# BaptisteHudyma/RGB-D-SLAM

Hardware: AMD Instinct MI355X
Metric: depth frames/s primitive extraction (640x480) (higher is better)
Workload: dtype f64; 1 GPU; 640x480 synthetic planar-room depth stream, plane extraction only (BASELINE.json configs[1]); stream_frames=4096, unique_frames_per_gpu=4096, scene=room, sub_batches=0, frames_rendered_on=device (torch)

## Files before the change

### profiles/a1_inventory.py

```python
#!/usr/bin/env python3
import argparse
import os
import subprocess
import sys

sys.path.insert(0, os.path.dirname(os.path.abspath(__file__)))
from valu_issue import CSRC, RATE_NS, classify, kernel_regions

SYMBOLS = (("f32", "_ZN4cape24cape_cell_moments_kernelILb0EEEvNS_12StageAParamsEi"),
           ("u16", "_ZN4cape24cape_cell_moments_kernelILb1EEEvNS_12StageAParamsEi"))
NAMES = {"prologue": "prologue", "loop_rows_0_9": "rows 0..9, one trip", "row_10": "row 10", "loop_rows_11_18": "rows 11..18, one trip",
         "tail": "tail", "redo_listed": "scan f64 redo"}
ORDER = tuple(NAMES)
WEIGHT = {"prologue": 1, "loop_rows_0_9": 10, "row_10": 1, "loop_rows_11_18": 8, "tail": 1, "redo_listed": 0}


def count(ops):
    c = {"f64": 0, "double_rate": 0, "other": 0}
    for op in ops:
        if op.startswith("v_"):
            c[classify(op)] += 1
    return c


def inventory(asm):
    return {variant: {name: count(ops) for name, ops in kernel_regions(asm, symbol)} for variant, symbol in SYMBOLS}


def priced(c):
# ... 31 lines not shown
```

### profiles/valu_issue.py

```python
#!/usr/bin/env python3
import argparse
import csv
import json
import os
import re
import subprocess
import sys

ROOT = os.path.dirname(os.path.dirname(os.path.abspath(__file__)))
CSRC = os.path.join(ROOT, "rgb-d-slam_amd", "csrc")

RATE_NS = {"f64": 1.95, "other": 1.85, "double_rate": 0.95}
DOUBLE_RATE = {"v_mul_f32", "v_add_f32", "v_sub_f32", "v_subrev_f32", "v_add_u32", "v_sub_u32", "v_subrev_u32", "v_and_b32", "v_mov_b32"}


def classify(op):
    base = re.sub(r"_(e32|e64|dpp|sdwa)$", "", op)
    if "f64" in base or base.endswith("_b64") and base.startswith("v_mov"):
        return "f64"
    if base in DOUBLE_RATE:
        return "double_rate"
    return "other"


def kernel_regions(asm_lines, symbol):
    start = next(i for i, ln in enumerate(asm_lines) if ln.startswith(symbol + ":"))
    end = next(i for i in range(start, len(asm_lines)) if "s_endpgm" in asm_lines[i])
    body = asm_lines[start + 1:end + 1]
    label_at = {m.group(1): i for i, ln in enumerate(body) for m in [re.match(r"^(\.LBB\d+_\d+):", ln)] if m}
    loops = []
    for i, ln in enumerate(body):
        m = re.match(r"\s+s_c?branch\w*\s+(\.LBB\d+_\d+)", ln)
        if m and label_at.get(m.group(1), len(body)) < i:
            loops.append((label_at[m.group(1)], i))
    assert len(loops) == 2, "two row loops"
    redo = []

    def ops(lo, hi):
        out, skip_to = [], None
        for ln in body[lo:hi]:
            if skip_to is not None:
                if ln.startswith(skip_to + ":"):
                    skip_to = None
                else:
                    m = re.match(r"\s+([vs]_\w+)", ln)
                    if m:
                        redo.append(m.group(1))
                    continue
            m = re.match(r"\s+([vs]_\w+|ds_\w+|global_\w+|buffer_\w+|flat_\w+|scratch_\w+)", ln)
            if m:
                out.append(m.group(1))
                v = re.match(r"\s+s_cbranch_vccz\s+(\.LBB\d+_\d+)", ln)
                if v:
                    skip_to = v.group(1)
        return out

    (h1, e1), (h2, e2) = loops
    regions = [("prologue", ops(0, h1)), ("loop_rows_0_9", ops(h1, e1 + 1)), ("row_10", ops(e1 + 1, h2)), ("loop_rows_11_18", ops(h2, e2 + 1)),
               ("tail", ops(e2 + 1, len(body)))]
    return regions + [("redo_listed", redo)]


def count(ops):
    c = {"f64": 0, "double_rate": 0, "other": 0, "salu": 0, "lds": 0, "vmem": 0}
    for op in ops:
        if op.startswith("v_"):
            c[classify(op)] += 1
        elif op.startswith("s_"):
            c["salu"] += 1
        elif op.startswith("ds_"):
            c["lds"] += 1
        else:
            c["vmem"] += 1
    return c
# ... 8 lines not shown
    ap.add_argument("--simds", type=int, default=1024)
    ap.add_argument("--out", default=os.path.join(ROOT, "profiles", "valu_issue.json"))
    args = ap.parse_args()

    asm_path = "/tmp/cape_cell_moments.gfx950.s"
    flags = "-O3 -std=c++17 -fPIC --offload-arch=gfx950 -ffp-contract=off -fno-fast-math -fno-slp-vectorize".split()
    subprocess.check_call(["/opt/rocm/bin/hipcc"] + flags + ["-S", "--cuda-device-only", "-o", asm_path, os.path.join(CSRC, "cape_cell_moments.hip")],
                          stderr=subprocess.DEVNULL)
    asm = open(asm_path).read().splitlines()
    cell = 20
    cells = (args.height // cell) * (args.width // cell)
    waves_per_launch = args.frames * ((cells + 63) // 64)
    out = {"kernel": "cape_cell_moments_kernel", "frames_per_launch": args.frames, "width": args.width, "height": args.height,
           "waves_per_launch": waves_per_launch, "simds": args.simds, "rate_ns_per_wave_instruction": RATE_NS,
           "rates_from": "profiles/r02_valu_rates.txt (csrc/microbench/valu_rates.hip on MI355X)", "variants": {}}
    for variant, symbol in (("f32", "_ZN4cape24cape_cell_moments_kernelILb0EEEvNS_12StageAParamsEi"),
                            ("u16", "_ZN4cape24cape_cell_moments_kernelILb1EEEvNS_12StageAParamsEi")):
        regs = dict(kernel_regions(asm, symbol))
        c = {k: count(v) for k, v in regs.items()}
        weights = {"prologue": 1, "loop_rows_0_9": cell // 2, "row_10": 1, "loop_rows_11_18": cell // 2 - 2, "tail": 1}
        per_wave = {k: sum(c[r][k] * w for r, w in weights.items()) for k in ("f64", "double_rate", "other", "salu", "lds", "vmem")}
        static_valu = per_wave["f64"] + per_wave["double_rate"] + per_wave["other"]
        v = {"static_per_wave": {"all_rows": per_wave, "per_region": {r: c[r] for r in weights}, "redo_listed_not_run": c["redo_listed"],
                                 "per_20_pixels_row_trip": c["loop_rows_0_9"]}}
        valu = static_valu
        if args.pmc:
            for row in csv.DictReader(open(args.pmc)):
                if ("cell_moments_kernel<false>" if variant == "f32" else "cell_moments_kernel<true>") in row["kernel"] and row["counter"] == "SQ_INSTS_VALU":
                    dyn = float(row["avg_value"])
                    v["pmc"] = {"SQ_INSTS_VALU_per_launch": dyn, "per_wave": dyn / waves_per_launch, "static_per_wave": static_valu,
                                "source": os.path.relpath(args.pmc, ROOT)}
                    valu = dyn / waves_per_launch
        mix = {k: per_wave[k] / max(1, static_valu) for k in RATE_NS}
        per_wave_ns = valu * sum(mix[k] * RATE_NS[k] for k in RATE_NS)
        floor_ms = per_wave_ns * waves_per_launch / args.simds * 1e-6
        f64_ns = valu * mix["f64"] * RATE_NS["f64"]
        v.update({"valu_per_wave": valu, "issue_ns_per_wave": per_wave_ns, "floor_ms": floor_ms,
                  "f64_rate_share_of_floor": f64_ns / per_wave_ns,
                  "f64_rate_insts_per_launch": valu * mix["f64"] * waves_per_launch,
                  "other_insts_per_launch": valu * (1.0 - mix["f64"]) * waves_per_launch})
        out["variants"][variant] = v
        print(f"{variant}: per wave (64 cells) f64-rate {per_wave['f64']}, double-rate {per_wave['double_rate']}, other {per_wave['other']} "
              f"= {static_valu} listed, {valu:.0f} priced ({valu / 5:.0f} per 80 pixels per lane); issue floor {floor_ms:.3f} ms per {args.frames} frames "
# ... 8 lines not shown
```

### rgb-d-slam_amd/csrc/cape_api.hip

```cpp
#include <algorithm>
#include <cmath>
#include <cstdlib>
#include <cstring>
#include <initializer_list>
#include <memory>
#include <new>
#include <random>
#include <string>
#include <vector>

#include "cape_handle.h"

using namespace cape::abi;

namespace {

thread_local std::string g_lastError;

constexpr int kRngTableMin = 40000;
int rng_table_size(int cells) { const int need = 43 * cells + 129; return need > kRngTableMin ? need : kRngTableMin; }

std::vector<double> rng_table(uint32_t seed, int count)
{
    std::vector<double> rng((size_t)count);
// ... 15 lines not shown
    const double det = (c00 * m[0][0] + c10 * m[1][0]) + c20 * m[2][0];
    const double invdet = 1.0 / det;
    k00 = c00 * invdet;
    k02 = c20 * invdet;
    k11 = cof(1, 1) * invdet;
    k12 = cof(2, 1) * invdet;
}

struct Knobs
{
    std::string resume;
    bool noResume = false;
    int schedule = 0;
    std::string stageA;
    std::string a1;
    bool growGeneral = false;
    bool pinnedByDma = false;
    int a2WideBatch = 0;
    int generalSlots = 0;
};

int read_knobs(Knobs& k)
{
    auto one_of = [](const char* name, std::initializer_list<const char*> values, std::string& out) {
        const char* e = std::getenv(name);
        if (!e)
            return true;
        out = e;
        return std::any_of(values.begin(), values.end(), [&](const char* v) { return out == v; });
    };
    std::string schedule, grow;
    if (!one_of("CAPE_RESUME", {"off", "wave", "group"}, k.resume))
        return fail(CAPE_ERR_INVALID_ARGUMENT, "CAPE_RESUME must be off, wave or group");
    if (!one_of("CAPE_SCHEDULE", {"two", "single"}, schedule))
        return fail(CAPE_ERR_INVALID_ARGUMENT, "CAPE_SCHEDULE must be two or single");
    if (!one_of("CAPE_STAGE_A", {"strips", "bands"}, k.stageA))
        return fail(CAPE_ERR_INVALID_ARGUMENT, "CAPE_STAGE_A must be strips or bands");
    if (!one_of("CAPE_A1", {"cells", "bands"}, k.a1))
        return fail(CAPE_ERR_INVALID_ARGUMENT, "CAPE_A1 must be cells or bands");
    if (!one_of("CAPE_GROW", {"general", "fast"}, grow))
        return fail(CAPE_ERR_INVALID_ARGUMENT, "CAPE_GROW must be general or fast");
    k.noResume = k.resume == "off" || std::getenv("CAPE_NO_RESUME");
    k.schedule = schedule == "two" ? 1 : (schedule == "single" ? 2 : 0);
    k.growGeneral = grow == "general";
    const char* e = std::getenv("CAPE_PINNED_INPUT");
    k.pinnedByDma = e && std::string(e) == "dma";
    if ((e = std::getenv("CAPE_A2_WIDE_BATCH")))
        k.a2WideBatch = std::atoi(e);
    if ((e = std::getenv("CAPE_GENERAL_SLOTS")))
        k.generalSlots = std::max(1, std::atoi(e));
    return CAPE_OK;
}

template <typename NextFn> int log_frame(cape_log_fn fn, void* user, const cape_frame_record& r, int frame, NextFn next)
// ... 294 lines not shown
    a.brow = h->brow;
    a.ratio_col = h->ratioCol;
    a.ratio_row = h->ratioRow;
    a.cell_sums = h->cellSums;
    a.cell_plane = h->cellPlane;
    a.cell_score = h->cellScore;
    a.cell_tol = h->cellTol;
    a.cell_flags = h->cellFlags;
    a.cell_bins = h->cellBins;
    a.cell_aux = h->cellAux;
    a.cell_mse = h->cellMse;
    a.sinMerge = sinf(static_cast<float>(18.0f * M_PI / 180.0));
    a.cosMergeA = std::cos(static_cast<double>(18.0f) * M_PI / 180.0);
    a.smallBatchFrames = knobs.a2WideBatch;
    a.a1Bands = knobs.a1 == "bands" ? 1 : 0;
    a.minZeroPointCount = static_cast<int>(std::floor(static_cast<float>(400) * 0.7f));

    cape::StageBParams& b = h->pb;
    b.W = cfg->width;
    b.H = cfg->height;
    b.hCells = h->hCells;
    b.vCells = h->vCells;
    b.cells = h->cells;
    b.acol = h->acol;
    b.brow = h->brow;
    b.cell_sums = h->cellSums;
    b.cell_plane = h->cellPlane;
    b.cell_score = h->cellScore;
    b.cell_tol = h->cellTol;
    b.cell_flags = h->cellFlags;
// ... 240 lines not shown
```

### rgb-d-slam_amd/csrc/cape_api_extract.hip

```cpp
#include <algorithm>
#include <atomic>
#include <chrono>
#include <cmath>
#include <cstring>

#include "cape_handle.h"

using namespace cape::abi;

namespace {

__global__ void cape_signal_kernel(uint32_t* flag, uint32_t seq)
{
    __hip_atomic_store(flag, seq, __ATOMIC_RELEASE, __HIP_MEMORY_SCOPE_SYSTEM);
}

void offset_params(const cape_handle_s* h, int f0, cape::StageAParams& a, cape::StageBParams& b)
{
    a = h->pa;
    b = h->pb;
    const size_t C = (size_t)h->cells, F = (size_t)f0;
    const size_t px = F * (size_t)h->cfg.width * h->cfg.height;
    if (a.depth)
        a.depth += px;
// ... 89 lines not shown
    if (t)
        CAPE_HIP_TRY(hipEventRecord(t->e[0], st));
    const bool strips = c.stripCounters && frames <= kHostResultFrames && (!c.inputOverLink || c.stripsAlways);
    cape::StageAParams a2 = a;
    cape::StageBParams bb = b;
    prepare_launch(h, a2, bb, c.spillCounters, strips, frames, t != nullptr);
    if (strips)
    {
        CAPE_HIP_TRY(cape::launch_cell_strips(a2, frames, c.stripCounters, st));
        if (t)
        {
            CAPE_HIP_TRY(hipEventRecord(t->e[1], st));
            CAPE_HIP_TRY(hipEventRecord(t->e[2], st));
        }
    }
    else
    {
        CAPE_HIP_TRY(cape::launch_cell_moments(a, frames, st));
        if (t)
            CAPE_HIP_TRY(hipEventRecord(t->e[1], st));
        CAPE_HIP_TRY(cape::launch_cell_plane(a2, frames, st));
        if (t)
            CAPE_HIP_TRY(hipEventRecord(t->e[2], st));
    }
    const bool oneFrameChain = h->resultsOnHost && r.doneFlag && r.doneCounter && frames <= kHostResultFrames;
    if (oneFrameChain)
    {
        bb.allFrames = c.generalAll ? 0 : 1;
        bb.doneFlag = r.doneFlag;
        bb.doneCounter = r.doneCounter;
// ... 403 lines not shown
```

### rgb-d-slam_amd/csrc/cape_cell_acc.h

```cpp
#pragma once
#include <hip/hip_runtime.h>

#include "cape_device.h"
#include "cape_internal.h"

namespace cape {


#ifndef CAPE_A_GROUP
#define CAPE_A_GROUP 2
#endif
#ifndef CAPE_A_WAVES
#define CAPE_A_WAVES 4
#endif

#ifndef CAPE_A1_CELL_WAVES
#define CAPE_A1_CELL_WAVES 4
#endif
#ifndef CAPE_A1_CELL_THREADS
#define CAPE_A1_CELL_THREADS 256
#endif
#ifndef CAPE_A1_CELL_LOAD_POLICY
#define CAPE_A1_CELL_LOAD_POLICY 0
#endif
constexpr int kThreadsCells = CAPE_A1_CELL_THREADS;
static_assert(kThreadsCells % 64 == 0 && kThreadsCells >= 64 && kThreadsCells <= 1024, "whole waves");

constexpr int kThreadsA = 320;
constexpr int kBandThreads = 160;
[[maybe_unused]] constexpr int kPartStride = 11;

struct PxAcc
// ... 94 lines not shown
```

### rgb-d-slam_amd/csrc/cape_cell_fit.hip

```cpp
#include <hip/hip_runtime.h>

#include <type_traits>

#include "cape_cell_acc.h"

namespace cape {

#ifndef CAPE_A2_WAVES
#define CAPE_A2_WAVES 4
#endif
#ifndef CAPE_A2_ABLATE
#define CAPE_A2_ABLATE 0
#endif
struct CellFit
{
    PlaneFit f;
    bool planar;
    float tol;
    int bin;
    uint32_t nearEdge, inorder, n;
    bool rewrite;
};
__device__ __forceinline__ void cell_fit_and_bin(const StageAParams& p, int frame, int cellRow, int cellCol, const CellAux& aux, double (&S)[9],
                                                 CellFit& o)
{
    PlaneFit f;
    f.planar = false;
    f.nx = f.ny = f.nz = f.d = 0.0;
    f.cx = f.cy = f.cz = 0.0;
    f.mse = kDblMax;
    f.score = 0.0;
    bool planar = false;
    float tol = 0.0f;
    int bin = -1;
    uint32_t nearEdge = 0, inorder = 0;
    uint32_t n = aux.flags & kCountMask;
    const bool continuous = (aux.flags & kAuxContinuous) != 0;
    const bool exact_ok = (aux.flags & kAuxExact) != 0;
    bool rewrite = false;
    if (!exact_ok && continuous && n >= (uint32_t)(kPts / 2))
    {
        inorder = 1;
        rewrite = true;
        const size_t cellOff = (size_t)frame * p.W * p.H + (size_t)(cellRow * kCell) * p.W + cellCol * kCell;
        PxAcc A;
#pragma unroll
        for (int k = 0; k < 9; ++k)
            A.S[k] = 0.0;
        A.n = 0;
        A.zminBits1 = 0;
        A.zmaxBits = 0;
        for (int r = 0; r < kCell; ++r)
        {
            const double b = p.brow[cellRow * kCell + r];
            for (int c = 0; c < kCell; ++c)
            {
                const size_t o = cellOff + (size_t)r * p.W + c;
                const float zr = p.depth ? p.depth[o] : (float)p.depth_u16[o] * p.u16_scale;
                acc_px(zr, p.acol[cellCol * kCell + c], b, A);
            }
        }
#pragma unroll
        for (int k = 0; k < 9; ++k)
            S[k] = A.S[k];
        n = A.n;
    }

    if (!continuous || n < (uint32_t)(kPts / 2))
    {
#pragma unroll
        for (int k = 0; k < 9; ++k)
            S[k] = 0.0;
        n = 0;
        rewrite = true;
    }
    else if (n >= (uint32_t)p.minZeroPointCount && !(CAPE_A2_ABLATE & 1))
    {
        fit_plane(S, n, f);
        const double qz = depth_quantization(f.cz);
        planar = f.mse <= qz * qz;
    }

    if ((CAPE_A2_ABLATE & 1) && n >= (uint32_t)p.minZeroPointCount)
    {
        planar = S[2] > 0.0;
        f.nx = S[0] * 1e-9, f.ny = S[1] * 1e-9, f.nz = -0.5, f.d = S[2] * 1e-6, f.cx = S[0] / n, f.cy = S[1] / n, f.cz = S[2] / n;
    }
    if (planar)
    {
        const float z0 = aux.z0, z1 = aux.z399;
        const int u0 = cellCol * kCell, v0 = cellRow * kCell;
        float x0 = 0, y0 = 0, zz0 = 0, x1 = 0, y1 = 0, zz1 = 0;
        if (z0 > 0)
        {
            x0 = (float)((double)z0 * p.acol[u0]);
            y0 = (float)((double)z0 * p.brow[v0]);
            zz0 = z0;
        }
        if (z1 > 0)
        {
            x1 = (float)((double)z1 * p.acol[u0 + kCell - 1]);
            y1 = (float)((double)z1 * p.brow[v0 + kCell - 1]);
            zz1 = z1;
        }
        const float dx = x1 - x0, dy = y1 - y0, dz = zz1 - zz0;
        const float diam = (CAPE_A2_ABLATE & 8) ? dx : sqrtf(dx * dx + (dy * dy + dz * dz));
        tol = (CAPE_A2_ABLATE & 8) ? diam : std_minf(50.0f, diam * p.sinMerge * sqrtf((float)n));

        const double theta = (CAPE_A2_ABLATE & 2) ? -f.nz : acos(-f.nz);
        const double phi = (CAPE_A2_ABLATE & 2) ? f.nx : atan2(f.nx, f.ny);
        constexpr double kPi = 3.14159265358979323846;
        const double tx = 19.0 * (theta - 0.0) / kPi;
        const int xQ = (int)floor(tx);
        int yQ = 0;
        double ty = 0.5;
        if (xQ > 0)
        {
            ty = 19.0 * (phi - (-kPi)) / (kPi - (-kPi));
            yQ = (int)floor(ty);
        }
        bin = yQ * 20 + xQ;
        if (fabs(tx - rint(tx)) < 1e-9 || (xQ > 0 && fabs(ty - rint(ty)) < 1e-9))
            nearEdge = 1;
    }
    o.f = f;
    o.planar = planar;
    o.tol = tol;
    o.bin = bin;
    o.nearEdge = nearEdge;
    o.inorder = inorder;
    o.n = n;
    o.rewrite = rewrite;
}

struct CellPub
{
    double nx, ny, nz, d, cx, cy, cz, tol;
};

template <int THREADS>
__global__ __launch_bounds__(THREADS, THREADS == 256 ? CAPE_A2_WAVES : 4) void cape_cell_plane_kernel(StageAParams p, int nFrames)
{
    __shared__ CellPub s_pub[THREADS];
    if (blockIdx.x == 0 && threadIdx.x == 0)
    {
        if (p.clear0)
            *p.clear0 = 0u;
        if (p.clear1)
            *p.clear1 = 0u;
        if (p.clear2)
        {
            *p.clear2 = 0u;
            if (p.clear2Buckets)
                for (int c = 1; c <= kResumeClasses; ++c)
                    p.clear2[(size_t)c * p.clear2Buckets] = 0u;
        }
        if (p.clear3)
            *p.clear3 = 0u;
        if (p.clear4)
            p.clear4[0] = p.clear4[1] = 0u;
    }
    const int HC = p.hCells, VC = p.vCells;
    const int rowsPerTile = THREADS / HC > 0 ? THREADS / HC : 1;
    const int tilesPerFrame = (VC + rowsPerTile - 1) / rowsPerTile;
    const int frame = blockIdx.x / tilesPerFrame;
    const int r0 = (blockIdx.x - frame * tilesPerFrame) * rowsPerTile;
    const int tid = threadIdx.x;
    const int tileCells = rowsPerTile * HC;
    const int lrow = tid / HC, cellCol = tid - lrow * HC;
    {
        const int cellRow = r0 + lrow;
        const bool valid = tid < tileCells && cellRow < VC;
        const int cell = cellRow * HC + cellCol;
        const size_t gcell = (size_t)frame * p.cells + (valid ? cell : 0);

        CellFit cf;
// ... 12 lines not shown
            const CellAux aux = p.cell_aux[gcell];
            double* os = p.cell_sums + gcell * kSumStride;
            double S[9];
#pragma unroll
            for (int k = 0; k < 9; ++k)
                S[k] = os[k];
            cell_fit_and_bin(p, frame, cellRow, cellCol, aux, S, cf);
            if (cf.rewrite)
            {
#pragma unroll
                for (int k = 0; k < 9; ++k)
                    os[k] = S[k];
                os[9] = (double)cf.n;
            }
        }
        const PlaneFit& f = cf.f;
        const bool planar = cf.planar;
        const float tol = cf.tol;
        const int bin = cf.bin;
        const uint32_t nearEdge = cf.nearEdge, inorder = cf.inorder, n = cf.n;

        CellPub me;
        me.nx = f.nx; me.ny = f.ny; me.nz = f.nz; me.d = f.d;
        me.cx = f.cx; me.cy = f.cy; me.cz = f.cz; me.tol = (double)tol;
        s_pub[tid] = me;
        __syncthreads();
        uint32_t edges = 0;
        if (valid)
        {
            if (cellCol > 0 && !(CAPE_A2_ABLATE & 4))
            {
                const CellPub L = s_pub[tid - 1];
                if (can_be_merged(L.nx, L.ny, L.nz, L.d, me.nx, me.ny, me.nz, me.cx, me.cy, me.cz, me.tol, p.cosMergeA))
                    edges |= kFlagLeftToMe;
                if (can_be_merged(me.nx, me.ny, me.nz, me.d, L.nx, L.ny, L.nz, L.cx, L.cy, L.cz, L.tol, p.cosMergeA))
                    edges |= kFlagMeToLeft;
            }
            if (lrow > 0 && !(CAPE_A2_ABLATE & 4))
            {
                const CellPub Up = s_pub[tid - HC];
                if (can_be_merged(Up.nx, Up.ny, Up.nz, Up.d, me.nx, me.ny, me.nz, me.cx, me.cy, me.cz, me.tol, p.cosMergeA))
                    edges |= kFlagUpToMe;
                if (can_be_merged(me.nx, me.ny, me.nz, me.d, Up.nx, Up.ny, Up.nz, Up.cx, Up.cy, Up.cz, Up.tol, p.cosMergeA))
                    edges |= kFlagMeToUp;
            }
            double* op = p.cell_plane + gcell * kPlaneStride;
            op[0] = f.nx; op[1] = f.ny; op[2] = f.nz; op[3] = f.d;
            op[4] = f.cx; op[5] = f.cy; op[6] = f.cz; op[7] = f.mse;
            p.cell_mse[gcell] = f.mse;
            p.cell_score[gcell] = f.score;
            p.cell_tol[gcell] = tol;
            p.cell_bins[gcell] = bin;
            p.cell_flags[gcell] = (n & kCountMask) | edges | (nearEdge ? kFlagNearEdge : 0u) | (inorder ? kFlagInorder : 0u) |
                                  (planar ? kFlagPlanar : 0u);
        }
    }
}

constexpr int kStripCells = 8;
constexpr int kStripThreads = 256;
constexpr int kStripCols = kStripCells * 5;
constexpr int kStripRowGroups = 5;
constexpr int kStripRows = kCell / kStripRowGroups;
constexpr int kStripActive = kStripCols * kStripRowGroups;
static_assert(kStripRows * kStripRowGroups == kCell && kStripActive <= kStripThreads, "strip geometry");

__device__ __forceinline__ float4 strip_to_f4(const float4& v, float) { return v; }
__device__ __forceinline__ float4 strip_to_f4(const ushort4& rw, float scale)
{
    auto mul1 = [](float a, float b) {
// ... 5 lines not shown
}

template <bool U16> __global__ __launch_bounds__(kStripThreads) void cape_cell_strip_kernel(StageAParams p, uint32_t* frameCounters)
{
    __shared__ double s_part[kStripActive * kPartStride];
    __shared__ float s_row[kStripCells * kCell];
    __shared__ float s_col[kStripCells * kCell];
    __shared__ float s_corner[kStripCells * 3];
    __shared__ double s_sum[kStripCells * 10];
    __shared__ uint32_t s_range[kStripCells * 2];
    __shared__ uint32_t s_cont[2 * kStripCells];
    __shared__ uint32_t s_last;

    const int t = threadIdx.x;
    if (blockIdx.x == 0 && t == 0)
    {
        if (p.clear0)
            *p.clear0 = 0u;
        if (p.clear1)
            *p.clear1 = 0u;
        if (p.clear2)
        {
            *p.clear2 = 0u;
            if (p.clear2Buckets)
                for (int c = 1; c <= kResumeClasses; ++c)
                    p.clear2[(size_t)c * p.clear2Buckets] = 0u;
        }
        if (p.clear3)
            *p.clear3 = 0u;
        if (p.clear4)
            p.clear4[0] = p.clear4[1] = 0u;
    }
    const int HC = p.hCells, VC = p.vCells;
    const int stripsPerRow = (HC + kStripCells - 1) / kStripCells;
    const int stripsPerFrame = stripsPerRow * VC;
    const int frame = blockIdx.x / stripsPerFrame;
    const int sidx = blockIdx.x - frame * stripsPerFrame;
    const int cellRow = sidx / stripsPerRow;
    const int strip = sidx - cellRow * stripsPerRow;
    const size_t frameOff = (size_t)frame * p.W * p.H;

    const int rg = t / kStripCols;
    const int q = t - rg * kStripCols;
    const int col0 = strip * (kStripCells * kCell) + q * 4;
    const bool active = t < kStripActive && col0 < p.W;
    const int cseg = q / 5, j = q - cseg * 5;

// ... 252 lines not shown
```

### rgb-d-slam_amd/csrc/cape_cell_moments.hip

```cpp
#include <hip/hip_runtime.h>

#include <type_traits>

#include "cape_cell_acc.h"

namespace cape {

template <bool U16> __global__ __launch_bounds__(kThreadsA, CAPE_A_WAVES) void cape_cell_moments_bands_kernel(StageAParams p)
{
    __shared__ double s_part[kThreadsA * kPartStride];
    __shared__ float s_row[64 * kCell];
    __shared__ float s_col[64 * kCell];
    __shared__ float s_corner[64 * 2];
    __shared__ float s_trash[kThreadsA + kCell];

    const int t = threadIdx.x;
    const int frame = blockIdx.x / p.pairsPerFrame;
    const int pair = blockIdx.x - frame * p.pairsPerFrame;
    const size_t frameOff = (size_t)frame * p.W * p.H;

    const int band0 = pair * 2;
    const int cellRow0 = band0 / p.segsPerRow;
    const int seg0 = band0 - cellRow0 * p.segsPerRow;
    const bool wrap = seg0 + 1 == p.segsPerRow;
// ... 221 lines not shown
        }
    }
    const float zmin = __uint_as_float(zminBits1 + 1u), zmax = __uint_as_float(zmaxBits);
    const float rab = fmaxf(p.ratio_col[fCol], p.ratio_row[fRow]);
    const bool exact_ok = zmaxBits <= 0x7F7FFFFFu && ((n == 0) || (zmax * rab <= 512.0f * zmin));

    const size_t gcell = (size_t)frame * p.cells + fRow * p.hCells + fCol;
    CellAux aux;
    aux.z0 = s_corner[c64 * 2];
    aux.z399 = s_corner[c64 * 2 + 1];
    aux.flags = (n & kCountMask) | (continuous ? kAuxContinuous : 0u) | (exact_ok ? kAuxExact : 0u);
    aux.zc = s_row[c64 * kCell + kCell / 2];
    p.cell_aux[gcell] = aux;
}

template <bool U16> __global__ __launch_bounds__(kThreadsCells, CAPE_A1_CELL_WAVES) void cape_cell_moments_kernel(StageAParams p, int nWaves)
{
    const int gw = __builtin_amdgcn_readfirstlane((int)(blockIdx.x * (kThreadsCells / 64) + (threadIdx.x >> 6)));
    if (gw >= nWaves)
        return;
    const int wavesPerFrame = (p.cells + 63) >> 6;
    const int frame = gw / wavesPerFrame;
    const int w = gw - frame * wavesPerFrame;
    const int cell = w * 64 + (int)(threadIdx.x & 63);
    if (cell >= p.cells)
        return;
    const int cellRow = cell / p.hCells;
    const int cellCol = cell - cellRow * p.hCells;
    const size_t frameOff = (size_t)frame * p.W * p.H;

    PxAcc A;
#pragma unroll
    for (int k = 0; k < 9; ++k)
        A.S[k] = 0.0;
    A.n = 0;
    A.zminBits1 = 0xFFFFFFFFu;
    A.zmaxBits = 0u;

    double a[kCell];
    {
        const double2* ap = reinterpret_cast<const double2*>(p.acol + cellCol * kCell);
// ... 135 lines not shown
#pragma unroll
    for (int j = 0; j < kQuads; ++j)
    {
        const float4 v = to_f4(buf[j]);
        acc_piece(v, j, b);
        z399 = v.w;
    }

    const uint32_t n = A.n;
    const float zmin = __uint_as_float(A.zminBits1 + 1u), zmax = __uint_as_float(A.zmaxBits);
    const size_t gcell = my_cell();
    const int ecell = (int)(gcell - (size_t)frame * p.cells);
    int hCells = p.hCells;
    asm volatile("" : "+s"(hCells));
    const int eRow = ecell / hCells;
    const float rab = fmaxf(p.ratio_col[ecell - eRow * hCells], p.ratio_row[eRow]);
    const bool exact_ok = A.zmaxBits <= 0x7F7FFFFFu && ((n == 0) || (zmax * rab <= 512.0f * zmin));

    CellAux aux;
    aux.z0 = z0;
    aux.z399 = z399;
    aux.flags = (n & kCountMask) | (continuous ? kAuxContinuous : 0u) | (exact_ok ? kAuxExact : 0u);
    aux.zc = zc;
    p.cell_aux[gcell] = aux;
    double2* dst = reinterpret_cast<double2*>(p.cell_sums + gcell * kSumStride);
    static_assert(kSumStride == 10, "nine sums and the count: five 16-B stores");
    dst[0] = make_double2(A.S[0], A.S[1]);
    dst[1] = make_double2(A.S[2], A.S[3]);
    dst[2] = make_double2(A.S[4], A.S[5]);
    dst[3] = make_double2(A.S[6], A.S[7]);
    dst[4] = make_double2(A.S[8], (double)n);
}

hipError_t launch_cell_moments(const StageAParams& p, int nFrames, hipStream_t stream)
{
    if (p.a1Bands)
    {
        const int grid = nFrames * p.pairsPerFrame;
        if (p.depth)
            hipLaunchKernelGGL(cape_cell_moments_bands_kernel<false>, dim3(grid), dim3(kThreadsA), 0, stream, p);
        else
            hipLaunchKernelGGL(cape_cell_moments_bands_kernel<true>, dim3(grid), dim3(kThreadsA), 0, stream, p);
        return hipGetLastError();
    }
    constexpr int kWaves = kThreadsCells / 64;
    const int waves = nFrames * ((p.cells + 63) / 64);
    const int grid = (waves + kWaves - 1) / kWaves;
    if (p.depth)
        hipLaunchKernelGGL(cape_cell_moments_kernel<false>, dim3(grid), dim3(kThreadsCells), 0, stream, p, waves);
    else
        hipLaunchKernelGGL(cape_cell_moments_kernel<true>, dim3(grid), dim3(kThreadsCells), 0, stream, p, waves);
    return hipGetLastError();
}

}
```

### rgb-d-slam_amd/csrc/cape_handle.h

```cpp
#pragma once

#include <hip/hip_runtime.h>

#include <cstring>
#include <string>
#include <utility>
#include <vector>

#include "cape_internal.h"

namespace cape {
hipError_t launch_cell_moments(const StageAParams& p, int nFrames, hipStream_t stream);
hipError_t launch_cell_plane(const StageAParams& p, int nFrames, hipStream_t stream);
hipError_t launch_cell_strips(const StageAParams& p, int nFrames, uint32_t* frameCounters, hipStream_t stream);
int cell_plane_rows_per_tile(const StageAParams& p, int nFrames);
hipError_t launch_grow(const StageBParams& p, int nFrames, hipStream_t stream, hipStream_t side, hipEvent_t fork, hipEvent_t done,
                       const GenParams* gen);
hipError_t launch_grow_general(const StageBParams& p, const GenParams& g, int nFrames, hipStream_t stream);
size_t grow_lds_bytes(int cells, bool cylinders, int maxPlanes);
size_t grow_state_bytes(int cells);
bool resume_group_fits(const StageBParams& p);
hipError_t launch_rectify(const RectifyParams& p, int nFrames, int computeUnits, hipStream_t stream);
hipError_t launch_match(const MatchParams& p, int nFrames, hipStream_t stream);
hipError_t launch_pack(const PackParams& p, hipStream_t stream);
hipError_t launch_polygons(const PolygonParams& p, int nFrames, hipStream_t stream);
hipError_t launch_match_polygons(const MatchPolygonParams& p, int nFrames, hipStream_t stream);
hipError_t launch_match_map(const MatchMapParams& p, int nFrames, hipStream_t stream);
hipError_t launch_match_map_wide(const MatchMapParams& p, int nFrames, hipStream_t stream);
hipError_t launch_match_wide(const MatchWideParams& p, int nFrames, hipStream_t stream);
hipError_t launch_carry_save(const CarrySaveParams& p, hipStream_t stream);
// ... 480 lines not shown
```

### rgb-d-slam_amd/csrc/cape_internal.h

```cpp
#pragma once
#include <stdint.h>

#include "../../include/cape_hip.h"

namespace cape {

constexpr int kSumStride = 10;
constexpr int kFastPlanes = 32;
constexpr int kProfileSlots = 32;
constexpr int kResumeClasses = 8;
constexpr int kCylStride = 8;
constexpr int kPlaneStride = 8;
constexpr uint32_t kFlagPlanar = 1u << 31;
constexpr uint32_t kFlagInorder = 1u << 30;
constexpr uint32_t kFlagNearEdge = 1u << 29;
constexpr uint32_t kCountMask = (1u << 24) - 1;
constexpr uint32_t kFlagLeftToMe = 1u << 24;
constexpr uint32_t kFlagMeToLeft = 1u << 25;
constexpr uint32_t kFlagUpToMe = 1u << 26;
constexpr uint32_t kFlagMeToUp = 1u << 27;
constexpr uint32_t kAuxContinuous = 1u << 31;
constexpr uint32_t kAuxExact = 1u << 30;

struct CellAux
// ... 22 lines not shown
    float* cell_tol;
    uint32_t* cell_flags;
    int32_t* cell_bins;
    CellAux* cell_aux;
    double* cell_mse;
    float sinMerge;
    uint32_t* clear0;
    uint32_t* clear1;
    uint32_t* clear2;
    uint32_t clear2Buckets;
    uint32_t* clear3;
    uint32_t* clear4;
    double cosMergeA;
    int smallBatchFrames;
    int a1Bands;
    int minZeroPointCount;
};

struct StageBParams
{
    int W, H, hCells, vCells, cells;
    const double* acol;
    const double* brow;
    const double* cell_sums;
    const double* cell_plane;
    const double* cell_score;
    const float* cell_tol;
    const uint32_t* cell_flags;
    const int32_t* cell_bins;
    const CellAux* cell_aux;
// ... 341 lines not shown
```

Baseline: 2.582 million frames/s.

## Fuse cell moments and per-cell plane fit into one kernel by default

Adds a fused path where the cell-moments kernel also fits the plane, computes the bin and tolerance, and evaluates neighbour merge edges through LDS. The split cell_plane launch and the round trip of per-cell sums through global memory are skipped. The fused path is taken by default when the grid of 256 cells per workgroup covers whole cell rows (a 32x24 grid fits). In exchange the kernel has more live registers and a block-wide barrier, and the early returns for out-of-range cells are removed.

```diff
diff --git a/profiles/a1_inventory.py b/profiles/a1_inventory.py
--- a/profiles/a1_inventory.py
+++ b/profiles/a1_inventory.py
@@ -7,12 +7,12 @@
 sys.path.insert(0, os.path.dirname(os.path.abspath(__file__)))
 from valu_issue import CSRC, RATE_NS, classify, kernel_regions
 
-SYMBOLS = (("f32", "_ZN4cape24cape_cell_moments_kernelILb0EEEvNS_12StageAParamsEi"),
-           ("u16", "_ZN4cape24cape_cell_moments_kernelILb1EEEvNS_12StageAParamsEi"))
+SYMBOLS = (("f32", "_ZN4cape24cape_cell_moments_kernelILb0ELb1EEEvNS_12StageAParamsEi"),
+           ("u16", "_ZN4cape24cape_cell_moments_kernelILb1ELb1EEEvNS_12StageAParamsEi"))
 NAMES = {"prologue": "prologue", "loop_rows_0_9": "rows 0..9, one trip", "row_10": "row 10", "loop_rows_11_18": "rows 11..18, one trip",
-         "tail": "tail", "redo_listed": "scan f64 redo"}
+         "tail": "tail", "fit_edges_writes": "fit + edges + stores (listed once)", "redo_listed": "scan f64 redo"}
 ORDER = tuple(NAMES)
-WEIGHT = {"prologue": 1, "loop_rows_0_9": 10, "row_10": 1, "loop_rows_11_18": 8, "tail": 1, "redo_listed": 0}
+WEIGHT = {"prologue": 1, "loop_rows_0_9": 10, "row_10": 1, "loop_rows_11_18": 8, "tail": 1, "fit_edges_writes": 1, "redo_listed": 0}
 
 
 def count(ops):
diff --git a/profiles/valu_issue.py b/profiles/valu_issue.py
--- a/profiles/valu_issue.py
+++ b/profiles/valu_issue.py
@@ -33,7 +33,8 @@
         m = re.match(r"\s+s_c?branch\w*\s+(\.LBB\d+_\d+)", ln)
         if m and label_at.get(m.group(1), len(body)) < i:
             loops.append((label_at[m.group(1)], i))
-    assert len(loops) == 2, "two row loops"
+    loops.sort()
+    assert len(loops) >= 2, "two row loops"
     redo = []
 
     def ops(lo, hi):
@@ -55,9 +56,10 @@
                     skip_to = v.group(1)
         return out
 
-    (h1, e1), (h2, e2) = loops
+    (h1, e1), (h2, e2) = loops[:2]
+    aux = next(i for i in range(e2 + 1, len(body)) if "global_store_dwordx4" in body[i])
     regions = [("prologue", ops(0, h1)), ("loop_rows_0_9", ops(h1, e1 + 1)), ("row_10", ops(e1 + 1, h2)), ("loop_rows_11_18", ops(h2, e2 + 1)),
-               ("tail", ops(e2 + 1, len(body)))]
+               ("tail", ops(e2 + 1, aux + 1)), ("fit_edges_writes", ops(aux + 1, len(body)))]
     return regions + [("redo_listed", redo)]
 
 
@@ -96,11 +98,11 @@
     out = {"kernel": "cape_cell_moments_kernel", "frames_per_launch": args.frames, "width": args.width, "height": args.height,
            "waves_per_launch": waves_per_launch, "simds": args.simds, "rate_ns_per_wave_instruction": RATE_NS,
            "rates_from": "profiles/r02_valu_rates.txt (csrc/microbench/valu_rates.hip on MI355X)", "variants": {}}
-    for variant, symbol in (("f32", "_ZN4cape24cape_cell_moments_kernelILb0EEEvNS_12StageAParamsEi"),
-                            ("u16", "_ZN4cape24cape_cell_moments_kernelILb1EEEvNS_12StageAParamsEi")):
+    for variant, symbol in (("f32", "_ZN4cape24cape_cell_moments_kernelILb0ELb1EEEvNS_12StageAParamsEi"),
+                            ("u16", "_ZN4cape24cape_cell_moments_kernelILb1ELb1EEEvNS_12StageAParamsEi")):
         regs = dict(kernel_regions(asm, symbol))
         c = {k: count(v) for k, v in regs.items()}
-        weights = {"prologue": 1, "loop_rows_0_9": cell // 2, "row_10": 1, "loop_rows_11_18": cell // 2 - 2, "tail": 1}
+        weights = {"prologue": 1, "loop_rows_0_9": cell // 2, "row_10": 1, "loop_rows_11_18": cell // 2 - 2, "tail": 1, "fit_edges_writes": 1}
         per_wave = {k: sum(c[r][k] * w for r, w in weights.items()) for k in ("f64", "double_rate", "other", "salu", "lds", "vmem")}
         static_valu = per_wave["f64"] + per_wave["double_rate"] + per_wave["other"]
         v = {"static_per_wave": {"all_rows": per_wave, "per_region": {r: c[r] for r in weights}, "redo_listed_not_run": c["redo_listed"],
@@ -108,7 +110,7 @@
         valu = static_valu
         if args.pmc:
             for row in csv.DictReader(open(args.pmc)):
-                if ("cell_moments_kernel<false>" if variant == "f32" else "cell_moments_kernel<true>") in row["kernel"] and row["counter"] == "SQ_INSTS_VALU":
+                if ("cell_moments_kernel<false, true>" if variant == "f32" else "cell_moments_kernel<true, true>") in row["kernel"] and row["counter"] == "SQ_INSTS_VALU":
                     dyn = float(row["avg_value"])
                     v["pmc"] = {"SQ_INSTS_VALU_per_launch": dyn, "per_wave": dyn / waves_per_launch, "static_per_wave": static_valu,
                                 "source": os.path.relpath(args.pmc, ROOT)}
diff --git a/rgb-d-slam_amd/csrc/cape_api.hip b/rgb-d-slam_amd/csrc/cape_api.hip
--- a/rgb-d-slam_amd/csrc/cape_api.hip
+++ b/rgb-d-slam_amd/csrc/cape_api.hip
@@ -53,6 +53,7 @@
     int schedule = 0;
     std::string stageA;
     std::string a1;
+    std::string a2;
     bool growGeneral = false;
     bool pinnedByDma = false;
     int a2WideBatch = 0;
@@ -77,6 +78,8 @@
         return fail(CAPE_ERR_INVALID_ARGUMENT, "CAPE_STAGE_A must be strips or bands");
     if (!one_of("CAPE_A1", {"cells", "bands"}, k.a1))
         return fail(CAPE_ERR_INVALID_ARGUMENT, "CAPE_A1 must be cells or bands");
+    if (!one_of("CAPE_A2", {"split", "fused"}, k.a2))
+        return fail(CAPE_ERR_INVALID_ARGUMENT, "CAPE_A2 must be split or fused");
     if (!one_of("CAPE_GROW", {"general", "fast"}, grow))
         return fail(CAPE_ERR_INVALID_ARGUMENT, "CAPE_GROW must be general or fast");
     k.noResume = k.resume == "off" || std::getenv("CAPE_NO_RESUME");
@@ -401,6 +404,12 @@
     a.cosMergeA = std::cos(static_cast<double>(18.0f) * M_PI / 180.0);
     a.smallBatchFrames = knobs.a2WideBatch;
     a.a1Bands = knobs.a1 == "bands" ? 1 : 0;
+    a.a2Fused = (knobs.a2 != "split" && !a.a1Bands && cape::cell_fused_eligible(a)) ? 1 : 0;
+    if (knobs.a2 == "fused" && (!a.a2Fused || knobs.a2WideBatch > 0 || cfg->sub_batches > 1))
+        return fail(CAPE_ERR_INVALID_ARGUMENT,
+                    "CAPE_A2=fused: this handle's grid of " + std::to_string(h->hCells) + " x " + std::to_string(h->vCells) +
+                        " cells is not eligible (256 cells per workgroup must be whole cell rows and divide the frame), or CAPE_A1=bands, "
+                        "CAPE_A2_WIDE_BATCH or sub_batches > 1 select the split kernels");
     a.minZeroPointCount = static_cast<int>(std::floor(static_cast<float>(400) * 0.7f));
 
     cape::StageBParams& b = h->pb;
diff --git a/rgb-d-slam_amd/csrc/cape_api_extract.hip b/rgb-d-slam_amd/csrc/cape_api_extract.hip
--- a/rgb-d-slam_amd/csrc/cape_api_extract.hip
+++ b/rgb-d-slam_amd/csrc/cape_api_extract.hip
@@ -127,6 +127,15 @@
             CAPE_HIP_TRY(hipEventRecord(t->e[2], st));
         }
     }
+    else if (a.a2Fused && cape::cell_plane_threads(a2, frames) == 256)
+    {
+        CAPE_HIP_TRY(cape::launch_cell_fused(a2, frames, st));
+        if (t)
+        {
+            CAPE_HIP_TRY(hipEventRecord(t->e[1], st));
+            CAPE_HIP_TRY(hipEventRecord(t->e[2], st));
+        }
+    }
     else
     {
         CAPE_HIP_TRY(cape::launch_cell_moments(a, frames, st));
diff --git a/rgb-d-slam_amd/csrc/cape_cell_acc.h b/rgb-d-slam_amd/csrc/cape_cell_acc.h
--- a/rgb-d-slam_amd/csrc/cape_cell_acc.h
+++ b/rgb-d-slam_amd/csrc/cape_cell_acc.h
@@ -16,6 +16,9 @@
 
 #ifndef CAPE_A1_CELL_WAVES
 #define CAPE_A1_CELL_WAVES 4
+#endif
+#ifndef CAPE_A1_FUSED_WAVES
+#define CAPE_A1_FUSED_WAVES 4
 #endif
 #ifndef CAPE_A1_CELL_THREADS
 #define CAPE_A1_CELL_THREADS 256
diff --git a/rgb-d-slam_amd/csrc/cape_cell_fit.hip b/rgb-d-slam_amd/csrc/cape_cell_fit.hip
--- a/rgb-d-slam_amd/csrc/cape_cell_fit.hip
+++ b/rgb-d-slam_amd/csrc/cape_cell_fit.hip
@@ -2,164 +2,20 @@
 
 #include <type_traits>
 
-#include "cape_cell_acc.h"
+#include "cape_cell_plane.h"
 
 namespace cape {
 
 #ifndef CAPE_A2_WAVES
 #define CAPE_A2_WAVES 4
 #endif
-#ifndef CAPE_A2_ABLATE
-#define CAPE_A2_ABLATE 0
-#endif
-struct CellFit
-{
-    PlaneFit f;
-    bool planar;
-    float tol;
-    int bin;
-    uint32_t nearEdge, inorder, n;
-    bool rewrite;
-};
-__device__ __forceinline__ void cell_fit_and_bin(const StageAParams& p, int frame, int cellRow, int cellCol, const CellAux& aux, double (&S)[9],
-                                                 CellFit& o)
-{
-    PlaneFit f;
-    f.planar = false;
-    f.nx = f.ny = f.nz = f.d = 0.0;
-    f.cx = f.cy = f.cz = 0.0;
-    f.mse = kDblMax;
-    f.score = 0.0;
-    bool planar = false;
-    float tol = 0.0f;
-    int bin = -1;
-    uint32_t nearEdge = 0, inorder = 0;
-    uint32_t n = aux.flags & kCountMask;
-    const bool continuous = (aux.flags & kAuxContinuous) != 0;
-    const bool exact_ok = (aux.flags & kAuxExact) != 0;
-    bool rewrite = false;
-    if (!exact_ok && continuous && n >= (uint32_t)(kPts / 2))
-    {
-        inorder = 1;
-        rewrite = true;
-        const size_t cellOff = (size_t)frame * p.W * p.H + (size_t)(cellRow * kCell) * p.W + cellCol * kCell;
-        PxAcc A;
-#pragma unroll
-        for (int k = 0; k < 9; ++k)
-            A.S[k] = 0.0;
-        A.n = 0;
-        A.zminBits1 = 0;
-        A.zmaxBits = 0;
-        for (int r = 0; r < kCell; ++r)
-        {
-            const double b = p.brow[cellRow * kCell + r];
-            for (int c = 0; c < kCell; ++c)
-            {
-                const size_t o = cellOff + (size_t)r * p.W + c;
-                const float zr = p.depth ? p.depth[o] : (float)p.depth_u16[o] * p.u16_scale;
-                acc_px(zr, p.acol[cellCol * kCell + c], b, A);
-            }
-        }
-#pragma unroll
-        for (int k = 0; k < 9; ++k)
-            S[k] = A.S[k];
-        n = A.n;
-    }
-
-    if (!continuous || n < (uint32_t)(kPts / 2))
-    {
-#pragma unroll
-        for (int k = 0; k < 9; ++k)
-            S[k] = 0.0;
-        n = 0;
-        rewrite = true;
-    }
-    else if (n >= (uint32_t)p.minZeroPointCount && !(CAPE_A2_ABLATE & 1))
-    {
-        fit_plane(S, n, f);
-        const double qz = depth_quantization(f.cz);
-        planar = f.mse <= qz * qz;
-    }
-
-    if ((CAPE_A2_ABLATE & 1) && n >= (uint32_t)p.minZeroPointCount)
-    {
-        planar = S[2] > 0.0;
-        f.nx = S[0] * 1e-9, f.ny = S[1] * 1e-9, f.nz = -0.5, f.d = S[2] * 1e-6, f.cx = S[0] / n, f.cy = S[1] / n, f.cz = S[2] / n;
-    }
-    if (planar)
-    {
-        const float z0 = aux.z0, z1 = aux.z399;
-        const int u0 = cellCol * kCell, v0 = cellRow * kCell;
-        float x0 = 0, y0 = 0, zz0 = 0, x1 = 0, y1 = 0, zz1 = 0;
-        if (z0 > 0)
-        {
-            x0 = (float)((double)z0 * p.acol[u0]);
-            y0 = (float)((double)z0 * p.brow[v0]);
-            zz0 = z0;
-        }
-        if (z1 > 0)
-        {
-            x1 = (float)((double)z1 * p.acol[u0 + kCell - 1]);
-            y1 = (float)((double)z1 * p.brow[v0 + kCell - 1]);
-            zz1 = z1;
-        }
-        const float dx = x1 - x0, dy = y1 - y0, dz = zz1 - zz0;
-        const float diam = (CAPE_A2_ABLATE & 8) ? dx : sqrtf(dx * dx + (dy * dy + dz * dz));
-        tol = (CAPE_A2_ABLATE & 8) ? diam : std_minf(50.0f, diam * p.sinMerge * sqrtf((float)n));
-
-        const double theta = (CAPE_A2_ABLATE & 2) ? -f.nz : acos(-f.nz);
-        const double phi = (CAPE_A2_ABLATE & 2) ? f.nx : atan2(f.nx, f.ny);
-        constexpr double kPi = 3.14159265358979323846;
-        const double tx = 19.0 * (theta - 0.0) / kPi;
-        const int xQ = (int)floor(tx);
-        int yQ = 0;
-        double ty = 0.5;
-        if (xQ > 0)
-        {
-            ty = 19.0 * (phi - (-kPi)) / (kPi - (-kPi));
-            yQ = (int)floor(ty);
-        }
-        bin = yQ * 20 + xQ;
-        if (fabs(tx - rint(tx)) < 1e-9 || (xQ > 0 && fabs(ty - rint(ty)) < 1e-9))
-            nearEdge = 1;
-    }
-    o.f = f;
-    o.planar = planar;
-    o.tol = tol;
-    o.bin = bin;
-    o.nearEdge = nearEdge;
-    o.inorder = inorder;
-    o.n = n;
-    o.rewrite = rewrite;
-}
-
-struct CellPub
-{
-    double nx, ny, nz, d, cx, cy, cz, tol;
-};
 
 template <int THREADS>
 __global__ __launch_bounds__(THREADS, THREADS == 256 ? CAPE_A2_WAVES : 4) void cape_cell_plane_kernel(StageAParams p, int nFrames)
 {
     __shared__ CellPub s_pub[THREADS];
     if (blockIdx.x == 0 && threadIdx.x == 0)
-    {
-        if (p.clear0)
-            *p.clear0 = 0u;
-        if (p.clear1)
-            *p.clear1 = 0u;
-        if (p.clear2)
-        {
-            *p.clear2 = 0u;
-            if (p.clear2Buckets)
-                for (int c = 1; c <= kResumeClasses; ++c)
-                    p.clear2[(size_t)c * p.clear2Buckets] = 0u;
-        }
-        if (p.clear3)
-            *p.clear3 = 0u;
-        if (p.clear4)
-            p.clear4[0] = p.clear4[1] = 0u;
-    }
+        clear_grow_counters(p);
     const int HC = p.hCells, VC = p.vCells;
     const int rowsPerTile = THREADS / HC > 0 ? THREADS / HC : 1;
     const int tilesPerFrame = (VC + rowsPerTile - 1) / rowsPerTile;
@@ -202,46 +58,7 @@
                 os[9] = (double)cf.n;
             }
         }
-        const PlaneFit& f = cf.f;
-        const bool planar = cf.planar;
-        const float tol = cf.tol;
-        const int bin = cf.bin;
-        const uint32_t nearEdge = cf.nearEdge, inorder = cf.inorder, n = cf.n;
-
-        CellPub me;
-        me.nx = f.nx; me.ny = f.ny; me.nz = f.nz; me.d = f.d;
-        me.cx = f.cx; me.cy = f.cy; me.cz = f.cz; me.tol = (double)tol;
-        s_pub[tid] = me;
-        __syncthreads();
-        uint32_t edges = 0;
-        if (valid)
-        {
-            if (cellCol > 0 && !(CAPE_A2_ABLATE & 4))
-            {
-                const CellPub L = s_pub[tid - 1];
-                if (can_be_merged(L.nx, L.ny, L.nz, L.d, me.nx, me.ny, me.nz, me.cx, me.cy, me.cz, me.tol, p.cosMergeA))
-                    edges |= kFlagLeftToMe;
-                if (can_be_merged(me.nx, me.ny, me.nz, me.d, L.nx, L.ny, L.nz, L.cx, L.cy, L.cz, L.tol, p.cosMergeA))
-                    edges |= kFlagMeToLeft;
-            }
-            if (lrow > 0 && !(CAPE_A2_ABLATE & 4))
-            {
-                const CellPub Up = s_pub[tid - HC];
-                if (can_be_merged(Up.nx, Up.ny, Up.nz, Up.d, me.nx, me.ny, me.nz, me.cx, me.cy, me.cz, me.tol, p.cosMergeA))
-                    edges |= kFlagUpToMe;
-                if (can_be_merged(me.nx, me.ny, me.nz, me.d, Up.nx, Up.ny, Up.nz, Up.cx, Up.cy, Up.cz, Up.tol, p.cosMergeA))
-                    edges |= kFlagMeToUp;
-            }
-            double* op = p.cell_plane + gcell * kPlaneStride;
-            op[0] = f.nx; op[1] = f.ny; op[2] = f.nz; op[3] = f.d;
-            op[4] = f.cx; op[5] = f.cy; op[6] = f.cz; op[7] = f.mse;
-            p.cell_mse[gcell] = f.mse;
-            p.cell_score[gcell] = f.score;
-            p.cell_tol[gcell] = tol;
-            p.cell_bins[gcell] = bin;
-            p.cell_flags[gcell] = (n & kCountMask) | edges | (nearEdge ? kFlagNearEdge : 0u) | (inorder ? kFlagInorder : 0u) |
-                                  (planar ? kFlagPlanar : 0u);
-        }
+        tile_publish_and_finish(p, s_pub, tid, HC, lrow, cellCol, valid, gcell, cf);
     }
 }
 
@@ -277,23 +94,7 @@
 
     const int t = threadIdx.x;
     if (blockIdx.x == 0 && t == 0)
-    {
-        if (p.clear0)
-            *p.clear0 = 0u;
-        if (p.clear1)
-            *p.clear1 = 0u;
-        if (p.clear2)
-        {
-            *p.clear2 = 0u;
-            if (p.clear2Buckets)
-                for (int c = 1; c <= kResumeClasses; ++c)
-                    p.clear2[(size_t)c * p.clear2Buckets] = 0u;
-        }
-        if (p.clear3)
-            *p.clear3 = 0u;
-        if (p.clear4)
-            p.clear4[0] = p.clear4[1] = 0u;
-    }
+        clear_grow_counters(p);
     const int HC = p.hCells, VC = p.vCells;
     const int stripsPerRow = (HC + kStripCells - 1) / kStripCells;
     const int stripsPerFrame = stripsPerRow * VC;
diff --git a/rgb-d-slam_amd/csrc/cape_cell_moments.hip b/rgb-d-slam_amd/csrc/cape_cell_moments.hip
--- a/rgb-d-slam_amd/csrc/cape_cell_moments.hip
+++ b/rgb-d-slam_amd/csrc/cape_cell_moments.hip
@@ -2,7 +2,7 @@
 
 #include <type_traits>
 
-#include "cape_cell_acc.h"
+#include "cape_cell_plane.h"
 
 namespace cape {
 
@@ -259,17 +259,20 @@
     p.cell_aux[gcell] = aux;
 }
 
-template <bool U16> __global__ __launch_bounds__(kThreadsCells, CAPE_A1_CELL_WAVES) void cape_cell_moments_kernel(StageAParams p, int nWaves)
+template <bool U16, bool FUSED>
+__global__ __launch_bounds__(kThreadsCells, FUSED ? CAPE_A1_FUSED_WAVES : CAPE_A1_CELL_WAVES) void cape_cell_moments_kernel(StageAParams p, int nWaves)
 {
     const int gw = __builtin_amdgcn_readfirstlane((int)(blockIdx.x * (kThreadsCells / 64) + (threadIdx.x >> 6)));
-    if (gw >= nWaves)
-        return;
+    if constexpr (!FUSED)
+        if (gw >= nWaves)
+            return;
     const int wavesPerFrame = (p.cells + 63) >> 6;
     const int frame = gw / wavesPerFrame;
     const int w = gw - frame * wavesPerFrame;
     const int cell = w * 64 + (int)(threadIdx.x & 63);
-    if (cell >= p.cells)
-        return;
+    if constexpr (!FUSED)
+        if (cell >= p.cells)
+            return;
     const int cellRow = cell / p.hCells;
     const int cellCol = cell - cellRow * p.hCells;
     const size_t frameOff = (size_t)frame * p.W * p.H;
@@ -435,7 +438,8 @@
     int hCells = p.hCells;
     asm volatile("" : "+s"(hCells));
     const int eRow = ecell / hCells;
-    const float rab = fmaxf(p.ratio_col[ecell - eRow * hCells], p.ratio_row[eRow]);
+    const int eCol = ecell - eRow * hCells;
+    const float rab = fmaxf(p.ratio_col[eCol], p.ratio_row[eRow]);
     const bool exact_ok = A.zmaxBits <= 0x7F7FFFFFu && ((n == 0) || (zmax * rab <= 512.0f * zmin));
 
     CellAux aux;
@@ -446,11 +450,47 @@
     p.cell_aux[gcell] = aux;
     double2* dst = reinterpret_cast<double2*>(p.cell_sums + gcell * kSumStride);
     static_assert(kSumStride == 10, "nine sums and the count: five 16-B stores");
-    dst[0] = make_double2(A.S[0], A.S[1]);
-    dst[1] = make_double2(A.S[2], A.S[3]);
-    dst[2] = make_double2(A.S[4], A.S[5]);
-    dst[3] = make_double2(A.S[6], A.S[7]);
-    dst[4] = make_double2(A.S[8], (double)n);
+    if constexpr (!FUSED)
+    {
+        dst[0] = make_double2(A.S[0], A.S[1]);
+        dst[1] = make_double2(A.S[2], A.S[3]);
+        dst[2] = make_double2(A.S[4], A.S[5]);
+        dst[3] = make_double2(A.S[6], A.S[7]);
+        dst[4] = make_double2(A.S[8], (double)n);
+    }
+    else
+    {
+        __shared__ CellPub s_pub[kThreadsCells];
+        const int tid = (int)((uint32_t)ecell % (uint32_t)kThreadsCells);
+        if (frame == 0 && ecell == 0)
+            clear_grow_counters(p);
+        CellFit cf;
+        cell_fit_and_bin(p, frame, eRow, eCol, aux, A.S, cf);
+        dst[0] = make_double2(A.S[0], A.S[1]);
+        dst[1] = make_double2(A.S[2], A.S[3]);
+        dst[2] = make_double2(A.S[4], A.S[5]);
+        dst[3] = make_double2(A.S[6], A.S[7]);
+        dst[4] = make_double2(A.S[8], (double)cf.n);
+        tile_publish_and_finish(p, s_pub, tid, hCells, tid / hCells, eCol, true, gcell, cf);
+    }
+}
+
+bool cell_fused_eligible(const StageAParams& p)
+{
+    return kThreadsCells == 256 && p.hCells > 0 && p.hCells <= 256 && 256 % p.hCells == 0 && p.cells % 256 == 0;
+}
+
+hipError_t launch_cell_fused(const StageAParams& p, int nFrames, hipStream_t stream)
+{
+    if (!cell_fused_eligible(p) || p.a1Bands)
+        return hipErrorInvalidConfiguration;
+    constexpr int kWaves = kThreadsCells / 64;
+    const int grid = nFrames * (p.cells / kThreadsCells);
+    if (p.depth)
+        hipLaunchKernelGGL((cape_cell_moments_kernel<false, true>), dim3(grid), dim3(kThreadsCells), 0, stream, p, grid * kWaves);
+    else
+        hipLaunchKernelGGL((cape_cell_moments_kernel<true, true>), dim3(grid), dim3(kThreadsCells), 0, stream, p, grid * kWaves);
+    return hipGetLastError();
 }
 
 hipError_t launch_cell_moments(const StageAParams& p, int nFrames, hipStream_t stream)
@@ -468,9 +508,9 @@
     const int waves = nFrames * ((p.cells + 63) / 64);
     const int grid = (waves + kWaves - 1) / kWaves;
     if (p.depth)
-        hipLaunchKernelGGL(cape_cell_moments_kernel<false>, dim3(grid), dim3(kThreadsCells), 0, stream, p, waves);
+        hipLaunchKernelGGL((cape_cell_moments_kernel<false, false>), dim3(grid), dim3(kThreadsCells), 0, stream, p, waves);
     else
-        hipLaunchKernelGGL(cape_cell_moments_kernel<true>, dim3(grid), dim3(kThreadsCells), 0, stream, p, waves);
+        hipLaunchKernelGGL((cape_cell_moments_kernel<true, false>), dim3(grid), dim3(kThreadsCells), 0, stream, p, waves);
     return hipGetLastError();
 }
 
diff --git a/rgb-d-slam_amd/csrc/cape_cell_plane.h b/rgb-d-slam_amd/csrc/cape_cell_plane.h
--- /dev/null
+++ b/rgb-d-slam_amd/csrc/cape_cell_plane.h
@@ -0,0 +1,201 @@
+#pragma once
+#include <hip/hip_runtime.h>
+
+#include "cape_cell_acc.h"
+
+namespace cape {
+
+#ifndef CAPE_A2_ABLATE
+#define CAPE_A2_ABLATE 0
+#endif
+struct CellFit
+{
+    PlaneFit f;
+    bool planar;
+    float tol;
+    int bin;
+    uint32_t nearEdge, inorder, n;
+    bool rewrite;
+};
+__device__ __forceinline__ void cell_fit_and_bin(const StageAParams& p, int frame, int cellRow, int cellCol, const CellAux& aux, double (&S)[9],
+                                                 CellFit& o)
+{
+    PlaneFit f;
+    f.planar = false;
+    f.nx = f.ny = f.nz = f.d = 0.0;
+    f.cx = f.cy = f.cz = 0.0;
+    f.mse = kDblMax;
+    f.score = 0.0;
+    bool planar = false;
+    float tol = 0.0f;
+    int bin = -1;
+    uint32_t nearEdge = 0, inorder = 0;
+    uint32_t n = aux.flags & kCountMask;
+    const bool continuous = (aux.flags & kAuxContinuous) != 0;
+    const bool exact_ok = (aux.flags & kAuxExact) != 0;
+    bool rewrite = false;
+    if (!exact_ok && continuous && n >= (uint32_t)(kPts / 2))
+    {
+        inorder = 1;
+        rewrite = true;
+        const size_t cellOff = (size_t)frame * p.W * p.H + (size_t)(cellRow * kCell) * p.W + cellCol * kCell;
+        PxAcc A;
+#pragma unroll
+        for (int k = 0; k < 9; ++k)
+            A.S[k] = 0.0;
+        A.n = 0;
+        A.zminBits1 = 0;
+        A.zmaxBits = 0;
+        for (int r = 0; r < kCell; ++r)
+        {
+            const double b = p.brow[cellRow * kCell + r];
+            for (int c = 0; c < kCell; ++c)
+            {
+                const size_t o = cellOff + (size_t)r * p.W + c;
+                const float zr = p.depth ? p.depth[o] : (float)p.depth_u16[o] * p.u16_scale;
+                acc_px(zr, p.acol[cellCol * kCell + c], b, A);
+            }
+        }
+#pragma unroll
+        for (int k = 0; k < 9; ++k)
+            S[k] = A.S[k];
+        n = A.n;
+    }
+
+    if (!continuous || n < (uint32_t)(kPts / 2))
+    {
+#pragma unroll
+        for (int k = 0; k < 9; ++k)
+            S[k] = 0.0;
+        n = 0;
+        rewrite = true;
+    }
+    else if (n >= (uint32_t)p.minZeroPointCount && !(CAPE_A2_ABLATE & 1))
+    {
+        fit_plane(S, n, f);
+        const double qz = depth_quantization(f.cz);
+        planar = f.mse <= qz * qz;
+    }
+
+    if ((CAPE_A2_ABLATE & 1) && n >= (uint32_t)p.minZeroPointCount)
+    {
+        planar = S[2] > 0.0;
+        f.nx = S[0] * 1e-9, f.ny = S[1] * 1e-9, f.nz = -0.5, f.d = S[2] * 1e-6, f.cx = S[0] / n, f.cy = S[1] / n, f.cz = S[2] / n;
+    }
+    if (planar)
+    {
+        const float z0 = aux.z0, z1 = aux.z399;
+        const int u0 = cellCol * kCell, v0 = cellRow * kCell;
+        float x0 = 0, y0 = 0, zz0 = 0, x1 = 0, y1 = 0, zz1 = 0;
+        if (z0 > 0)
+        {
+            x0 = (float)((double)z0 * p.acol[u0]);
+            y0 = (float)((double)z0 * p.brow[v0]);
+            zz0 = z0;
+        }
+        if (z1 > 0)
+        {
+            x1 = (float)((double)z1 * p.acol[u0 + kCell - 1]);
+            y1 = (float)((double)z1 * p.brow[v0 + kCell - 1]);
+            zz1 = z1;
+        }
+        const float dx = x1 - x0, dy = y1 - y0, dz = zz1 - zz0;
+        const float diam = (CAPE_A2_ABLATE & 8) ? dx : sqrtf(dx * dx + (dy * dy + dz * dz));
+        tol = (CAPE_A2_ABLATE & 8) ? diam : std_minf(50.0f, diam * p.sinMerge * sqrtf((float)n));
+
+        const double theta = (CAPE_A2_ABLATE & 2) ? -f.nz : acos(-f.nz);
+        const double phi = (CAPE_A2_ABLATE & 2) ? f.nx : atan2(f.nx, f.ny);
+        constexpr double kPi = 3.14159265358979323846;
+        const double tx = 19.0 * (theta - 0.0) / kPi;
+        const int xQ = (int)floor(tx);
+        int yQ = 0;
+        double ty = 0.5;
+        if (xQ > 0)
+        {
+            ty = 19.0 * (phi - (-kPi)) / (kPi - (-kPi));
+            yQ = (int)floor(ty);
+        }
+        bin = yQ * 20 + xQ;
+        if (fabs(tx - rint(tx)) < 1e-9 || (xQ > 0 && fabs(ty - rint(ty)) < 1e-9))
+            nearEdge = 1;
+    }
+    o.f = f;
+    o.planar = planar;
+    o.tol = tol;
+    o.bin = bin;
+    o.nearEdge = nearEdge;
+    o.inorder = inorder;
+    o.n = n;
+    o.rewrite = rewrite;
+}
+
+struct CellPub
+{
+    double nx, ny, nz, d, cx, cy, cz, tol;
+};
+
+__device__ __forceinline__ void tile_publish_and_finish(const StageAParams& p, CellPub* s_pub, int tid, int HC, int lrow, int cellCol, bool valid,
+                                                         size_t gcell, const CellFit& cf)
+{
+    const PlaneFit& f = cf.f;
+    const bool planar = cf.planar;
+    const float tol = cf.tol;
+    const int bin = cf.bin;
+    const uint32_t nearEdge = cf.nearEdge, inorder = cf.inorder, n = cf.n;
+
+    CellPub me;
+    me.nx = f.nx; me.ny = f.ny; me.nz = f.nz; me.d = f.d;
+    me.cx = f.cx; me.cy = f.cy; me.cz = f.cz; me.tol = (double)tol;
+    s_pub[tid] = me;
+    __syncthreads();
+    uint32_t edges = 0;
+    if (valid)
+    {
+        if (cellCol > 0 && !(CAPE_A2_ABLATE & 4))
+        {
+            const CellPub L = s_pub[tid - 1];
+            if (can_be_merged(L.nx, L.ny, L.nz, L.d, me.nx, me.ny, me.nz, me.cx, me.cy, me.cz, me.tol, p.cosMergeA))
+                edges |= kFlagLeftToMe;
+            if (can_be_merged(me.nx, me.ny, me.nz, me.d, L.nx, L.ny, L.nz, L.cx, L.cy, L.cz, L.tol, p.cosMergeA))
+                edges |= kFlagMeToLeft;
+        }
+        if (lrow > 0 && !(CAPE_A2_ABLATE & 4))
+        {
+            const CellPub Up = s_pub[tid - HC];
+            if (can_be_merged(Up.nx, Up.ny, Up.nz, Up.d, me.nx, me.ny, me.nz, me.cx, me.cy, me.cz, me.tol, p.cosMergeA))
+                edges |= kFlagUpToMe;
+            if (can_be_merged(me.nx, me.ny, me.nz, me.d, Up.nx, Up.ny, Up.nz, Up.cx, Up.cy, Up.cz, Up.tol, p.cosMergeA))
+                edges |= kFlagMeToUp;
+        }
+        double* op = p.cell_plane + gcell * kPlaneStride;
+        op[0] = f.nx; op[1] = f.ny; op[2] = f.nz; op[3] = f.d;
+        op[4] = f.cx; op[5] = f.cy; op[6] = f.cz; op[7] = f.mse;
+        p.cell_mse[gcell] = f.mse;
+        p.cell_score[gcell] = f.score;
+        p.cell_tol[gcell] = tol;
+        p.cell_bins[gcell] = bin;
+        p.cell_flags[gcell] = (n & kCountMask) | edges | (nearEdge ? kFlagNearEdge : 0u) | (inorder ? kFlagInorder : 0u) |
+                              (planar ? kFlagPlanar : 0u);
+    }
+}
+
+__device__ __forceinline__ void clear_grow_counters(const StageAParams& p)
+{
+    if (p.clear0)
+        *p.clear0 = 0u;
+    if (p.clear1)
+        *p.clear1 = 0u;
+    if (p.clear2)
+    {
+        *p.clear2 = 0u;
+        if (p.clear2Buckets)
+            for (int c = 1; c <= kResumeClasses; ++c)
+                p.clear2[(size_t)c * p.clear2Buckets] = 0u;
+    }
+    if (p.clear3)
+        *p.clear3 = 0u;
+    if (p.clear4)
+        p.clear4[0] = p.clear4[1] = 0u;
+}
+
+}
diff --git a/rgb-d-slam_amd/csrc/cape_handle.h b/rgb-d-slam_amd/csrc/cape_handle.h
--- a/rgb-d-slam_amd/csrc/cape_handle.h
+++ b/rgb-d-slam_amd/csrc/cape_handle.h
@@ -13,7 +13,10 @@
 hipError_t launch_cell_moments(const StageAParams& p, int nFrames, hipStream_t stream);
 hipError_t launch_cell_plane(const StageAParams& p, int nFrames, hipStream_t stream);
 hipError_t launch_cell_strips(const StageAParams& p, int nFrames, uint32_t* frameCounters, hipStream_t stream);
+int cell_plane_threads(const StageAParams& p, int nFrames);
 int cell_plane_rows_per_tile(const StageAParams& p, int nFrames);
+bool cell_fused_eligible(const StageAParams& p);
+hipError_t launch_cell_fused(const StageAParams& p, int nFrames, hipStream_t stream);
 hipError_t launch_grow(const StageBParams& p, int nFrames, hipStream_t stream, hipStream_t side, hipEvent_t fork, hipEvent_t done,
                        const GenParams* gen);
 hipError_t launch_grow_general(const StageBParams& p, const GenParams& g, int nFrames, hipStream_t stream);
diff --git a/rgb-d-slam_amd/csrc/cape_internal.h b/rgb-d-slam_amd/csrc/cape_internal.h
--- a/rgb-d-slam_amd/csrc/cape_internal.h
+++ b/rgb-d-slam_amd/csrc/cape_internal.h
@@ -60,6 +60,7 @@
     double cosMergeA;
     int smallBatchFrames;
     int a1Bands;
+    int a2Fused;
     int minZeroPointCount;
 };
 
```

Measured after the change: 2.679 million frames/s (median of 6 runs). +3.8%, better.
